# debbiemarkslab/BEAR

Hardware: AMD Instinct MI355X
Metric: k-mer contexts/sec (DM-marginal+grad h), k=13 (higher is better)
Workload: dtype f64

## Files before the change

bear_amd/csrc/bear_hip.hip:

```cpp
#include "bear_host.h"
#include "kernels_finalize.h"
#include "kernels_rows.h"
#include "kernels_sorted.h"
#include "kernels_plan.h"
#include "kernels_synth.h"
#include "kernels_refmix.h"
#include "kernels_mixplan.h"
#include "kernels_sample.h"
#include "kernels_shuffle.h"
#include "kernels_refplan.h"

#ifdef PLN_STAMPS
#define PLN_DBG_ARG , ws->dbg
#else
#define PLN_DBG_ARG
#endif

thread_local int g_last_hip_error = 0;

extern "C" {

int bear_abi_version(void) { return BEAR_ABI_VERSION; }

const char *bear_strerror(int status) {
// ... 648 lines not shown
  hipStream_t s = static_cast<hipStream_t>(stream);
  bear_params only_eps;
  memset(&only_eps, 0, sizeof(only_eps));
  only_eps.eps = eps;
  if (plan_is_rows(plan)) return launch_prior_rows(ws, plan, prior, only_eps, h_signed_dev, train_ar, out, grad_prior, s);
  if (grad_prior) return launch_prior_plan_grad(ws, plan, prior, only_eps, h_signed_dev, train_ar, prior_normalized, out, grad_prior, s);
  return launch_prior_plan(ws, plan, prior, n_rows, only_eps, h_signed_dev, train_ar, prior_normalized, out, s);
}

int bear_dm_refmix_plan_grad_f64(bear_ws *ws, const bear_plan *plan, const uint32_t *counts, const double *net_rows,
                                 const double *ref_rows, uint64_t n_rows, const double *h_signed_dev, const double *tau_signed_dev,
                                 const double *net_weight_signed_dev, double eps, int train_ar, double *out, double *grad_net_rows,
                                 void *stream) {
  int st = check_ws(ws);
  if (st != BEAR_OK) return st;
  if (!plan || !out || !h_signed_dev || !tau_signed_dev || !net_weight_signed_dev) return BEAR_ERR_INVALID_ARG;
  if (n_rows && (!counts || !net_rows || !ref_rows || !grad_net_rows)) return BEAR_ERR_INVALID_ARG;
  if (plan->ncol != 5 || plan->n_rows != n_rows || plan->counts != counts || plan->device != ws->device) return BEAR_ERR_INVALID_ARG;
  if (misaligned(net_rows) || misaligned(ref_rows) || misaligned(grad_net_rows) || misaligned8(out) || misaligned8(h_signed_dev) ||
      misaligned8(tau_signed_dev) || misaligned8(net_weight_signed_dev) || !(eps >= 0.0))
    return BEAR_ERR_INVALID_ARG;
  hipStream_t s = static_cast<hipStream_t>(stream);
  const int grid = grid_plan(ws, plan->n_tiles);
  const double2 *lt = reinterpret_cast<const double2 *>(ws->logtab);
  const pln_view pv = plan_view(plan);
  const bear_step_io io = ws_io(ws, nullptr, BEAR_THETA_REF, out);
  if (train_ar)
    hipLaunchKernelGGL(dm_refmix_plan_grad_kernel<true>, dim3(grid), dim3(PLN_THREADS), sizeof(pln_lds_g), s, net_rows, ref_rows,
                       h_signed_dev, tau_signed_dev, net_weight_signed_dev, eps, pv, lt, grad_net_rows, ws->partials, io);
  else
    hipLaunchKernelGGL(dm_refmix_plan_grad_kernel<false>, dim3(grid), dim3(PLN_THREADS), sizeof(pln_lds_g), s, net_rows, ref_rows,
                       h_signed_dev, tau_signed_dev, net_weight_signed_dev, eps, pv, lt, grad_net_rows, ws->partials, io);
  HIP_TRY(hipGetLastError());
  if (pv.n_heavy_col + pv.n_heavy_row) {
    const uint64_t nh = pv.n_heavy_col + pv.n_heavy_row;
    const int g2 = grid_capped((nh + 255) / 256, (uint64_t)ws->num_cu * 4);
    if (train_ar)
      hipLaunchKernelGGL(dm_refmix_fixup_kernel<true>, dim3(g2), dim3(256), 0, s, net_rows, ref_rows, h_signed_dev, tau_signed_dev,
                         net_weight_signed_dev, eps, pv, lt, grad_net_rows);
    else
      hipLaunchKernelGGL(dm_refmix_fixup_kernel<false>, dim3(g2), dim3(256), 0, s, net_rows, ref_rows, h_signed_dev, tau_signed_dev,
                         net_weight_signed_dev, eps, pv, lt, grad_net_rows);
    HIP_TRY(hipGetLastError());
  }
  return BEAR_OK;
}


static int launch_ref_plan(bear_ws *ws, const bear_plan *plan, const uint32_t *ref, uint64_t n_rows, const bear_params &prm,
                           const double *theta, int train_ar, double *out, hipStream_t s, const bear_apply_io &apply = NO_APPLY) {
  const double2 *lt = reinterpret_cast<const double2 *>(ws->logtab);
  const bear_step_io io = ws_io(ws, theta, BEAR_THETA_REF, out);
  int grid;
  if (plan->rows_ref) {
    if (plan->ref != ref) return BEAR_ERR_INVALID_ARG;
    grid = grid_dense(ws, n_rows);
    if (train_ar)
      hipLaunchKernelGGL(dm_ref_rows_kernel<true>, dim3(grid), dim3(BEAR_THREADS), 0, s, plan->counts, ref, n_rows, prm, lt, ws->partials, io, apply);
    else
      hipLaunchKernelGGL(dm_ref_rows_kernel<false>, dim3(grid), dim3(BEAR_THREADS), 0, s, plan->counts, ref, n_rows, prm, lt, ws->partials, io, apply);
  } else if (plan->ref) {
    if (plan->ref != ref) return BEAR_ERR_INVALID_ARG;
    rpl_view rv;
    rv.items = plan->ref_items;
    rv.n_items = plan->n_ref_items;
    rv.hist0 = plan->hist0;
    rv.heavy0 = plan->heavy0;
    rv.n_heavy0 = plan->n_heavy0;
    rv.sum0 = plan->sum0;
    const uint64_t units = (plan->n_ref_items + 63) / 64, want = (units + 3) / 4 + 2, cap = (uint64_t)ws->num_cu * (units > 131072 ? 6 : 4);
    grid = grid_capped(want, cap);
    if (train_ar)
      hipLaunchKernelGGL(dm_ref_items_kernel<true>, dim3(grid), dim3(256), 0, s, prm, rv, plan_view(plan), lt, ws->partials, io, apply);
    else
      hipLaunchKernelGGL(dm_ref_items_kernel<false>, dim3(grid), dim3(256), 0, s, prm, rv, plan_view(plan), lt, ws->partials, io, apply);
  } else {
    grid = grid_plan(ws, plan->n_tiles);
    if (train_ar)
      hipLaunchKernelGGL(dm_ref_plan_kernel<true>, dim3(grid), dim3(PLN_THREADS), sizeof(pln_lds_r), s, ref, n_rows, prm, plan_view(plan), lt,
                         ws->partials, io, apply);
    else
      hipLaunchKernelGGL(dm_ref_plan_kernel<false>, dim3(grid), dim3(PLN_THREADS), sizeof(pln_lds_r), s, ref, n_rows, prm, plan_view(plan), lt,
                         ws->partials, io, apply);
  }
  HIP_TRY(hipGetLastError());
  (void)grid;
  return BEAR_OK;
}

int bear_dm_ref_plan_f64(bear_ws *ws, const bear_plan *plan, const uint32_t *train, const uint32_t *ref,
                         uint64_t n_rows, double h_signed, double tau_signed, double nu_signed, double eps,
                         int train_ar, double *out, void *stream) {
  int st = check_ws(ws);
  if (st != BEAR_OK) return st;
  if (!plan || !out || (n_rows && (!train || !ref))) return BEAR_ERR_INVALID_ARG;
  if (plan->ncol != 4 || plan->n_rows != n_rows || plan->counts != train || plan->device != ws->device)
    return BEAR_ERR_INVALID_ARG;
  if (misaligned(ref) || (reinterpret_cast<uintptr_t>(out) & 7u)) return BEAR_ERR_INVALID_ARG;
  hipStream_t s = static_cast<hipStream_t>(stream);
  bear_params prm;
  const double tau = exp(tau_signed), nw = exp(nu_signed);
  prm.inv_h = 1.0 / exp(h_signed);
  prm.eps = eps;
  prm.E = exp(-tau);
  prm.tauE = tau * prm.E;
  prm.tau = tau;
  prm.V = 1.0 / (nw + 1.0);
  prm.nw = nw;
  return launch_ref_plan(ws, plan, ref, n_rows, prm, nullptr, train_ar, out, s);
}

int bear_ref_train_reduce_f64(bear_ws *ws, const bear_plan *plan, const uint32_t *train, const uint32_t *ref, uint64_t n_rows,
                              const double *theta, double eps, int train_ar, double *packed, void *stream) {
  int st = check_ws(ws);
  if (st != BEAR_OK) return st;
  if (!plan || !packed || !theta || !n_rows || !train || !ref) return BEAR_ERR_INVALID_ARG;
  if (plan->ncol != 4 || plan->n_rows != n_rows || plan->counts != train || plan->device != ws->device)
    return BEAR_ERR_INVALID_ARG;
  if (misaligned(ref) || (reinterpret_cast<uintptr_t>(packed) & 7u)) return BEAR_ERR_INVALID_ARG;
  hipStream_t s = static_cast<hipStream_t>(stream);
  bear_params only_eps;
  memset(&only_eps, 0, sizeof(only_eps));
  only_eps.eps = eps;
  return launch_ref_plan(ws, plan, ref, n_rows, only_eps, theta, train_ar, packed, s);
}

int bear_ref_train_step_f64(bear_ws *ws, const bear_plan *plan, const uint32_t *train, const uint32_t *ref, uint64_t n_rows,
                            double *theta, double *adam_m, double *adam_v, double *adam_t, double eps, int train_ar,
                            double learning_rate, double scale, double *out, double *loss_buf, uint64_t loss_cap, void *stream) {
  if (!adam_m || !adam_v || !adam_t) return BEAR_ERR_INVALID_ARG;
  if (two_launch_step()) {
    int st = bear_ref_train_reduce_f64(ws, plan, train, ref, n_rows, theta, eps, train_ar, out, stream);
    if (st != BEAR_OK) return st;
    return launch_train_apply(theta, 3, out, adam_m, adam_v, adam_t, learning_rate, scale, train_ar, loss_buf, loss_cap,
                              static_cast<hipStream_t>(stream));
  }
  int st = check_ws(ws);
  if (st != BEAR_OK) return st;
  if (!plan || !out || !theta || !n_rows || !train || !ref) return BEAR_ERR_INVALID_ARG;
  if (plan->ncol != 4 || plan->n_rows != n_rows || plan->counts != train || plan->device != ws->device) return BEAR_ERR_INVALID_ARG;
  if (misaligned(ref) || (reinterpret_cast<uintptr_t>(out) & 7u)) return BEAR_ERR_INVALID_ARG;
  bear_params only_eps;
  memset(&only_eps, 0, sizeof(only_eps));
  only_eps.eps = eps;
  return launch_ref_plan(ws, plan, ref, n_rows, only_eps, theta, train_ar, out, static_cast<hipStream_t>(stream),
                         make_apply(theta, 3, adam_m, adam_v, adam_t, learning_rate, scale, train_ar, loss_buf, loss_cap));
}

int bear_dm_items_f64(bear_ws *ws, const double *x, const uint32_t *c, uint64_t n, int path, double *D, double *P,
                      void *stream) {
  int st = check_ws(ws);
  if (st != BEAR_OK) return st;
  if (n == 0) return BEAR_OK;
  if (!x || !c || !D || !P || path < 0 || path > 2) return BEAR_ERR_INVALID_ARG;
  uint64_t blocks = (n + 255) / 256;
  if (blocks > 0x7fffffffull) return BEAR_ERR_INVALID_ARG;
  hipLaunchKernelGGL(dm_items_kernel, dim3((unsigned)blocks), dim3(256), 0, static_cast<hipStream_t>(stream), x, c, n, path,
                     reinterpret_cast<const double2 *>(ws->logtab), D, P);
  HIP_TRY(hipGetLastError());
  return BEAR_OK;
}

int bear_plan_count_total(const bear_plan *plan, double *total, double *bound) {
  if (!plan) return BEAR_ERR_INVALID_ARG;
  for (int k = 0; k < 3; ++k) {
    if (total) total[k] = plan->count_total[k];
    if (bound) bound[k] = plan->count_bound[k];
  }
  return BEAR_OK;
}

int bear_plan_set_count_bound(bear_plan *plan, const double *bound) {
  if (!plan || !bound) return BEAR_ERR_INVALID_ARG;
  for (int k = 0; k < 3; ++k)
    if (!(bound[k] >= plan->count_total[k]) || !(bound[k] < 0x1p50)) return BEAR_ERR_INVALID_ARG;
  for (int k = 0; k < 3; ++k) plan->count_bound[k] = bound[k];
  return BEAR_OK;
}

static int refmix_grid(const bear_ws *ws, uint64_t n_rows) { return grid_capped((n_rows + RMX_THREADS - 1) / RMX_THREADS, ws_blocks(ws, 2)); }

int bear_ref_mix_forward_f64(bear_ws *ws, const double *net_rows, const double *ref_rows, uint64_t n_rows, const double *tau_signed,
                             const double *net_weight_signed, double *prior, void *stream) {
  int st = check_ws(ws);
  if (st != BEAR_OK) return st;
  if (!tau_signed || !net_weight_signed || misaligned8(tau_signed) || misaligned8(net_weight_signed)) return BEAR_ERR_INVALID_ARG;
  if (n_rows == 0) return BEAR_OK;
  if (!net_rows || !ref_rows || !prior || misaligned(net_rows) || misaligned(ref_rows) || misaligned(prior)) return BEAR_ERR_INVALID_ARG;
  hipLaunchKernelGGL(ref_mix_forward_kernel, dim3(refmix_grid(ws, n_rows)), dim3(RMX_THREADS), 0, static_cast<hipStream_t>(stream),
                     net_rows, ref_rows, tau_signed, net_weight_signed, n_rows, prior);
  HIP_TRY(hipGetLastError());
  return BEAR_OK;
}

int bear_ref_mix_backward_f64(bear_ws *ws, const double *net_rows, const double *ref_rows, const double *grad_prior, uint64_t n_rows,
                              const double *tau_signed, const double *net_weight_signed, double *grad_net_rows, double *grad_scalars,
                              void *stream) {
  int st = check_ws(ws);
  if (st != BEAR_OK) return st;
  if (!tau_signed || !net_weight_signed || !grad_scalars || misaligned8(tau_signed) || misaligned8(net_weight_signed) ||
      misaligned8(grad_scalars))
    return BEAR_ERR_INVALID_ARG;
  hipStream_t s = static_cast<hipStream_t>(stream);
  if (n_rows == 0) {
    HIP_TRY(hipMemsetAsync(grad_scalars, 0, 2 * sizeof(double), s));
    return BEAR_OK;
  }
  if (!net_rows || !ref_rows || !grad_prior || !grad_net_rows || misaligned(net_rows) || misaligned(ref_rows) ||
      misaligned(grad_prior) || misaligned(grad_net_rows))
    return BEAR_ERR_INVALID_ARG;
  hipLaunchKernelGGL(ref_mix_backward_kernel, dim3(refmix_grid(ws, n_rows)), dim3(RMX_THREADS), 0, s, net_rows, ref_rows, grad_prior,
                     tau_signed, net_weight_signed, n_rows, grad_net_rows, ws->partials, ws_arrival(ws), grad_scalars);
  HIP_TRY(hipGetLastError());
  return BEAR_OK;
}

int bear_debug_read_timing(bear_ws *ws, unsigned long long *host, int n_words) {
  if (!ws || !host) return BEAR_ERR_INVALID_ARG;
  HIP_TRY(hipDeviceSynchronize());
  HIP_TRY(hipMemcpy(host, ws->dbg, sizeof(unsigned long long) * (size_t)n_words, hipMemcpyDeviceToHost));
  return BEAR_OK;
}

int bear_debug_occupancy(int which) {
  int nb = -1;
  hipError_t e = which == 0
      ? hipOccupancyMaxActiveBlocksPerMultiprocessor(&nb, dm_prior_sorted_kernel<0>, SRT_THREADS, sizeof(srt_lds_n))
      : hipOccupancyMaxActiveBlocksPerMultiprocessor(&nb, dm_ref_sorted_kernel, SRT_THREADS, sizeof(srt_lds_r));
  return e == hipSuccess ? nb : -1000 - (int)e;
}

int bear_log_gamma_f64(const double *conc, uint64_t n, uint64_t n_samples, uint64_t seed, double *out, void *stream) {
  if (n == 0 || n_samples == 0) return BEAR_OK;
  if (!conc || !out) return BEAR_ERR_INVALID_ARG;
  if (n_samples > (~0ull) / n) return BEAR_ERR_INVALID_ARG;
  const uint64_t total = n * n_samples;
  uint64_t blocks = (total + SMP_THREADS - 1) / SMP_THREADS;
  if (blocks > 65536) blocks = 65536;
  hipLaunchKernelGGL(log_gamma_kernel, dim3((unsigned)blocks), dim3(SMP_THREADS), 0, static_cast<hipStream_t>(stream), conc, n,
                     n_samples, seed, out);
  HIP_TRY(hipGetLastError());
  return BEAR_OK;
}

static int logdir_sample_launch(const uint32_t *counts, const double *prior, uint64_t n_rows, int width, const double *h,
                                int n_h, int with_ar, const double *van, int n_van, int mc_samples, int map, uint64_t seed,
                                uint64_t row_base, double *out, void *stream) {
  if (n_h < 0 || n_van < 0 || n_h + n_van > SMP_MAX_MODELS || (n_h && !h) || (n_van && !van)) return BEAR_ERR_INVALID_ARG;
  if (with_ar && !map) return BEAR_ERR_INVALID_ARG;
  if (map) mc_samples = 1;
  if (mc_samples <= 0) return BEAR_ERR_INVALID_ARG;
  const int M = (with_ar ? 1 : 0) + n_h + n_van;
  if (n_rows == 0 || M == 0) return BEAR_OK;
  if (!out || ((n_h || with_ar) && !prior)) return BEAR_ERR_INVALID_ARG;
  smp_args A;
  memset(&A, 0, sizeof(A));
  A.n_h = n_h;
  A.n_van = n_van;
  A.arm = with_ar ? 1 : 0;
  A.has_counts = counts ? 1 : 0;
  A.has_prior = prior ? 1 : 0;
  A.map = map ? 1 : 0;
  A.mc = (uint32_t)mc_samples;
  A.seed = seed;
  A.row_base = row_base;
  for (int j = 0; j < n_h; ++j) {
    if (!(h[j] > 0.0)) return BEAR_ERR_INVALID_ARG;
    A.w[j] = 1.0 / h[j];
  }
  for (int k = 0; k < n_van; ++k) A.w[n_h + k] = van[k];
  const uint64_t per_row = (uint64_t)M * (uint64_t)mc_samples;
  if (per_row > 0xffffffffull || n_rows > (~0ull) / ((uint64_t)width * per_row)) return BEAR_ERR_INVALID_ARG;
  uint64_t blocks = (n_rows * per_row + SMP_THREADS - 1) / SMP_THREADS;
  if (blocks > 65536) blocks = 65536;
  hipStream_t s = static_cast<hipStream_t>(stream);
  if (width == 21)
    hipLaunchKernelGGL(logdir_sample_kernel<21>, dim3((unsigned)blocks), dim3(SMP_THREADS), 0, s, counts, prior, n_rows, A, out);
  else
    hipLaunchKernelGGL(logdir_sample_kernel<5>, dim3((unsigned)blocks), dim3(SMP_THREADS), 0, s, counts, prior, n_rows, A, out);
  HIP_TRY(hipGetLastError());
  return BEAR_OK;
}

int bear_logdir_sample_f64(const uint32_t *counts, const double *prior, uint64_t n_rows, const double *h, int n_h,
                           int with_ar, const double *van, int n_van, int mc_samples, int map, uint64_t seed,
                           uint64_t row_base, double *out, void *stream) {
  return logdir_sample_launch(counts, prior, n_rows, 5, h, n_h, with_ar, van, n_van, mc_samples, map, seed, row_base, out, stream);
}

int bear_logdir_sample_wide_f64(const uint32_t *counts, const double *prior, uint64_t n_rows, int width, const double *h,
                                int n_h, int with_ar, const double *van, int n_van, int mc_samples, int map, uint64_t seed,
                                uint64_t row_base, double *out, void *stream) {
  if (!wide_width_ok(width)) return BEAR_ERR_INVALID_ARG;
  return logdir_sample_launch(counts, prior, n_rows, width, h, n_h, with_ar, van, n_van, mc_samples, map, seed, row_base, out,
                              stream);
}

int bear_shuffle_rows(const void *src, void *dst, uint64_t n_rows, uint32_t row_bytes, uint64_t seed, void *stream) {
  if (n_rows == 0 || row_bytes == 0) return BEAR_OK;
  if (!src || !dst || src == dst) return BEAR_ERR_INVALID_ARG;
  if (n_rows > (1ull << 62) / row_bytes) return BEAR_ERR_INVALID_ARG;
  const uint32_t hb = shf_half_bits(n_rows);
  const bool words = (row_bytes % 4 == 0) && ((reinterpret_cast<uintptr_t>(src) | reinterpret_cast<uintptr_t>(dst)) % 4 == 0);
  const uint64_t total = words ? n_rows * (row_bytes / 4) : n_rows * (uint64_t)row_bytes;
  uint64_t blocks = (total + 255) / 256;
  if (blocks > 1u << 20) blocks = 1u << 20;
  if (words)
    hipLaunchKernelGGL(shuffle_words_kernel, dim3((unsigned)blocks), dim3(256), 0, static_cast<hipStream_t>(stream),
                       static_cast<const uint32_t *>(src), static_cast<uint32_t *>(dst), n_rows, row_bytes / 4, hb, seed);
// ... 43 lines not shown
```

bear_amd/csrc/bear_math.h:

```cpp
#pragma once
#include <hip/hip_runtime.h>
#include <stdint.h>

#define BEAR_KPROD 16u
#define BEAR_TSTIR 8.0

struct bear_dp {
  double D;
  double P;
};

__device__ __forceinline__ double bear_rcp(double x) {
  double r = __builtin_amdgcn_rcp(x);
  double e = __builtin_fma(-x, r, 1.0);
  r = __builtin_fma(r, e, r);
  e = __builtin_fma(-x, r, 1.0);
  r = __builtin_fma(r, e, r);
  return r;
}

__device__ __forceinline__ double bear_log(double x) { return log(x); }

__device__ __forceinline__ double bear_log1p_pos(double t) {
  double u = 1.0 + t;
  double d = t - (u - 1.0);
  return bear_log(u) + d * bear_rcp(u);
}

__device__ __forceinline__ double bear_stir_lg(double r) {
  double r2 = r * r;
  double s = 1.0 / 156.0;
  s = __builtin_fma(s, r2, -691.0 / 360360.0);
  s = __builtin_fma(s, r2, 1.0 / 1188.0);
  s = __builtin_fma(s, r2, -1.0 / 1680.0);
  s = __builtin_fma(s, r2, 1.0 / 1260.0);
  s = __builtin_fma(s, r2, -1.0 / 360.0);
  s = __builtin_fma(s, r2, 1.0 / 12.0);
  return s * r;
}

__device__ __forceinline__ double bear_stir_psi(double r) {
  double r2 = r * r;
  double s = 1.0 / 12.0;
  s = __builtin_fma(s, r2, -691.0 / 32760.0);
  s = __builtin_fma(s, r2, 1.0 / 132.0);
  s = __builtin_fma(s, r2, -1.0 / 240.0);
  s = __builtin_fma(s, r2, 1.0 / 252.0);
  s = __builtin_fma(s, r2, -1.0 / 120.0);
  s = __builtin_fma(s, r2, 1.0 / 12.0);
  return s * r2;
}

__device__ __forceinline__ bear_dp bear_stirling_diff(double y, double c) {
  double y1 = y + c;
  double ry = bear_rcp(y), ry1 = bear_rcp(y1);
  double l1p = bear_log1p_pos(c * ry);
  double ly = bear_log(y);
  bear_dp o;
  o.D = __builtin_fma(y1 - 0.5, l1p, c * (ly - 1.0)) + (bear_stir_lg(ry1) - bear_stir_lg(ry));
  o.P = l1p - 0.5 * (ry1 - ry) - (bear_stir_psi(ry1) - bear_stir_psi(ry));
  return o;
}

__device__ __forceinline__ bear_dp bear_dm_item(double x, double c) {
  uint32_t m;
  if (c > (double)BEAR_KPROD || x > 0x1p60) {
    double need = BEAR_TSTIR - x;
    m = need > 0.0 ? (uint32_t)ceil(need) : 0u;
  } else {
    m = (uint32_t)c;
  }
  double p = 1.0, dp = 0.0, t = x;
  for (uint32_t j = 0; j < m; ++j) {
    dp = __builtin_fma(dp, t, p);
    p *= t;
    t += 1.0;
  }
  bear_dp o;
  o.D = 0.0;
  o.P = 0.0;
  if (m > 0) {
    o.D = bear_log(p);
    o.P = dp * bear_rcp(p);
  }
  if ((double)m < c) {
    bear_dp s = bear_stirling_diff(t, c - (double)m);
    o.D += s.D;
    o.P += s.P;
  }
  return o;
}

__device__ __forceinline__ double bear_fma3(double a, double b, double c) {
  double r;
  asm("v_fma_f64 %0, %1, %2, %3" : "=v"(r) : "v"(a), "v"(b), "v"(c));
  return r;
}
template <bool COEF_V = false>
__device__ __forceinline__ double bear_log1p_small(double t) {
  double q;
  if (COEF_V) asm("v_fma_f64 %0, %1, %2, %3" : "=v"(q) : "v"(-1.0 / 6.0), "v"(t), "v"(0.2));
  else asm("v_fma_f64 %0, %1, %2, %3" : "=v"(q) : "s"(-1.0 / 6.0), "v"(t), "v"(0.2));
  q = __builtin_fma(q, t, -0.25);
  q = bear_fma3(q, t, 1.0 / 3.0);
  q = __builtin_fma(q, t, -0.5);
  return __builtin_fma(t * t, q, t);
}

#define BEAR_LOGTAB_N 128
template <bool COEF_V = false>
__device__ __forceinline__ double bear_log_tab(double p, const double2 *__restrict__ tab) {
  const double m = __builtin_amdgcn_frexp_mant(p);
  const int e = __builtin_amdgcn_frexp_exp(p);
  const uint32_t hi = (uint32_t)(__double_as_longlong(m) >> 32);
  const double2 rl = tab[(hi >> 13) & 127u];
  const double t = __builtin_fma(m, rl.x, -1.0);
  const double l1p = bear_log1p_small<COEF_V>(t);
  return __builtin_fma((double)e, 0.6931471805599453094, rl.y + l1p);
}


__device__ __forceinline__ bear_dp bear_dm_item_fast(double x, double c, const double2 *__restrict__ tab) {
  uint32_t m;
  const bool stir = c > (double)BEAR_KPROD || x > 0x1p60;
  if (stir) {
    const double need = BEAR_TSTIR - x;
    m = need > 0.0 ? (uint32_t)ceil(need) : 0u;
  } else {
    m = (uint32_t)c;
  }
  double p = 1.0, dp = 0.0, t = x;
  for (uint32_t j = 0; j < m; ++j) {
    dp = __builtin_fma(dp, t, p);
    p *= t;
    t += 1.0;
  }
  bear_dp o;
  o.D = 0.0;
  o.P = 0.0;
  if (m > 0) {
    o.D = bear_log_tab(p, tab);
    o.P = dp * bear_rcp(p);
  }
  if (stir) {
    const double y = t, cc = c - (double)m, y1 = y + cc;
    const double ry = bear_rcp(y), ry1 = bear_rcp(y1);
    const double r = cc * ry;
    const double ly = bear_log_tab(y, tab);
    const double u1 = 1.0 + r;
    const double l1p = r < 0x1p-8 ? bear_log1p_small(r) : __builtin_fma(r - (u1 - 1.0), bear_rcp(u1), bear_log_tab(u1, tab));
    o.D += __builtin_fma(y1 - 0.5, l1p, cc * (ly - 1.0)) + (bear_stir_lg(ry1) - bear_stir_lg(ry));
    o.P += l1p - 0.5 * (ry1 - ry) - (bear_stir_psi(ry1) - bear_stir_psi(ry));
  }
  return o;
}

#define BEAR_EXPTAB_N 128
__device__ __forceinline__ double bear_exp_tab(double z, const double *__restrict__ tab) {
  if (z < -700.0) return 0.0;
  const double kf = __builtin_rint(z * 184.66496523378731);
  double r = __builtin_fma(kf, -0x1.62e42fee00000p-8, z);
  r = __builtin_fma(kf, -0x1.a39ef35793c76p-40, r);
  const int ki = (int)kf;
  const double t = tab[ki & (BEAR_EXPTAB_N - 1)];
  double p = __builtin_fma(r, 1.0 / 120.0, 1.0 / 24.0);
  p = __builtin_fma(r, p, 1.0 / 6.0);
  p = __builtin_fma(r, p, 0.5);
  p = __builtin_fma(r, p, 1.0);
  const double v = __builtin_fma(t, r * p, t);
  return __longlong_as_double(__double_as_longlong(v) + ((long long)(ki >> 7) << 52));
}

template <int CTRL>
__device__ __forceinline__ double bear_dpp_mov(double v) {
  const long long q = __double_as_longlong(v);
  const int lo = __builtin_amdgcn_mov_dpp((int)(uint32_t)q, CTRL, 0xf, 0xf, true);
  const int hi = __builtin_amdgcn_mov_dpp((int)(uint32_t)(q >> 32), CTRL, 0xf, 0xf, true);
  return __longlong_as_double(((long long)hi << 32) | (uint32_t)lo);
}
__device__ __forceinline__ double bear_wave_sum(double v) {
  v += bear_dpp_mov<0xB1>(v);
  v += bear_dpp_mov<0x4E>(v);
  v += bear_dpp_mov<0x124>(v);
  v += bear_dpp_mov<0x128>(v);
#pragma unroll
  for (int step = 0; step < 2; ++step) {
    const long long q = __double_as_longlong(v);
    const uint32_t lo = (uint32_t)q, hi = (uint32_t)(q >> 32);
    const auto a = step == 0 ? __builtin_amdgcn_permlane16_swap(lo, lo, false, false) : __builtin_amdgcn_permlane32_swap(lo, lo, false, false);
    const auto c = step == 0 ? __builtin_amdgcn_permlane16_swap(hi, hi, false, false) : __builtin_amdgcn_permlane32_swap(hi, hi, false, false);
    v = __longlong_as_double(((long long)c[0] << 32) | a[0]) + __longlong_as_double(((long long)c[1] << 32) | a[1]);
  }
  return v;
}
__device__ __forceinline__ double bear_wave_max(double v) {
  v = __builtin_fmax(v, bear_dpp_mov<0xB1>(v));
  v = __builtin_fmax(v, bear_dpp_mov<0x4E>(v));
  v = __builtin_fmax(v, bear_dpp_mov<0x124>(v));
  v = __builtin_fmax(v, bear_dpp_mov<0x128>(v));
#pragma unroll
  for (int step = 0; step < 2; ++step) {
    const long long q = __double_as_longlong(v);
    const uint32_t lo = (uint32_t)q, hi = (uint32_t)(q >> 32);
    const auto a = step == 0 ? __builtin_amdgcn_permlane16_swap(lo, lo, false, false) : __builtin_amdgcn_permlane32_swap(lo, lo, false, false);
    const auto c = step == 0 ? __builtin_amdgcn_permlane16_swap(hi, hi, false, false) : __builtin_amdgcn_permlane32_swap(hi, hi, false, false);
    v = __builtin_fmax(__longlong_as_double(((long long)c[0] << 32) | a[0]), __longlong_as_double(((long long)c[1] << 32) | a[1]));
  }
  return v;
}
```

bear_amd/csrc/kernels_rows.h:

```cpp
#pragma once
#include "bear_common.h"

__device__ __forceinline__ void stage_dwords(uint32_t *lds, const uint32_t *src, uint32_t n_dwords) {
  const uint32_t n_vec = n_dwords >> 2;
  const uint4 *s4 = reinterpret_cast<const uint4 *>(src);
  uint4 *d4 = reinterpret_cast<uint4 *>(lds);
  for (uint32_t i = threadIdx.x; i < n_vec; i += BEAR_THREADS) d4[i] = s4[i];
  for (uint32_t i = (n_vec << 2) + threadIdx.x; i < n_dwords; i += BEAR_THREADS) lds[i] = src[i];
}

__device__ __forceinline__ bear_dp dm_row_item(double x, double c, const double2 *tab) {
  if (tab && x > 0.0 && x < INFINITY) return bear_dm_item_fast(x, c, tab);
  return bear_dm_item(x, c);
}
__device__ __forceinline__ double dm_row(const uint32_t (&c)[5], const double (&a)[5], double (&g)[5], const double2 *tab = nullptr) {
  const double n = (((double)c[0] + (double)c[1]) + ((double)c[2] + (double)c[3])) + (double)c[4];
  double ll = 0.0;
#pragma unroll
  for (int b = 0; b < 5; ++b) g[b] = 0.0;
  if (n == 0.0) return 0.0;
  double A = ((a[0] + a[1]) + (a[2] + a[3])) + a[4];
  bear_dp tn = dm_row_item(A, n, tab);
  ll = -tn.D;
#pragma unroll
  for (int b = 0; b < 5; ++b) {
    g[b] = -tn.P;
    if (c[b] != 0) {
      bear_dp tb = dm_row_item(a[b], (double)c[b], tab);
      ll += tb.D;
      g[b] += tb.P;
    }
  }
  return ll;
}

template <bool AR, bool GRAD>
__global__ __launch_bounds__(BEAR_THREADS) void dm_prior_kernel(const uint32_t *__restrict__ counts,
                                                                 const double *__restrict__ prior,
                                                                 uint64_t n_rows, bear_params prm,
                                                                 double *__restrict__ grad_prior,
                                                                 const double2 *__restrict__ logtab_g,
                                                                 double *__restrict__ partials) {
  __shared__ __attribute__((aligned(16))) uint32_t s_cnt[BEAR_TILE_ROWS * 5];
  __shared__ __attribute__((aligned(16))) double s_pri[BEAR_TILE_ROWS * 5];
  __shared__ double2 s_log[BEAR_LOGTAB_N];
  if (threadIdx.x < BEAR_LOGTAB_N) s_log[threadIdx.x] = logtab_g[threadIdx.x];
  const uint64_t n_tiles = (n_rows + BEAR_TILE_ROWS - 1) / BEAR_TILE_ROWS;
  double acc[2] = {0.0, 0.0};
  for (uint64_t tile = blockIdx.x; tile < n_tiles; tile += gridDim.x) {
    const uint64_t row0 = tile * BEAR_TILE_ROWS;
    const uint32_t rows = (uint32_t)((n_rows - row0 < BEAR_TILE_ROWS) ? (n_rows - row0) : BEAR_TILE_ROWS);
    __syncthreads();
    stage_dwords(s_cnt, counts + row0 * 5, rows * 5);
    stage_dwords(reinterpret_cast<uint32_t *>(s_pri), reinterpret_cast<const uint32_t *>(prior + row0 * 5),
                 rows * 10);
    __syncthreads();
#pragma unroll 1
    for (int k = 0; k < BEAR_ROWS_PER_THREAD; ++k) {
      const uint32_t r = threadIdx.x + k * BEAR_THREADS;
      if (r >= rows) break;
      uint32_t c[5];
      double f[5];
#pragma unroll
      for (int b = 0; b < 5; ++b) {
        c[b] = s_cnt[r * 5 + b];
        f[b] = s_pri[r * 5 + b];
      }
      if (AR) {
#pragma unroll
        for (int b = 0; b < 5; ++b) {
          double p = f[b] + prm.eps;
          double cb = (double)c[b];
          if (c[b] != 0) acc[0] += cb * (p > 0.0 ? bear_log_tab(p, s_log) : bear_log(p));
          if (GRAD) grad_prior[(row0 + r) * 5 + b] = c[b] != 0 ? cb * bear_rcp(p) : 0.0;
        }
      } else {
        double a[5], g[5];
#pragma unroll
        for (int b = 0; b < 5; ++b) a[b] = __builtin_fma(f[b], prm.inv_h, prm.eps);
        acc[0] += dm_row(c, a, g, s_log);
        double dh = 0.0;
#pragma unroll
        for (int b = 0; b < 5; ++b) {
          dh = __builtin_fma(g[b], f[b], dh);
          if (GRAD) grad_prior[(row0 + r) * 5 + b] = g[b] * prm.inv_h;
        }
        acc[1] -= dh * prm.inv_h;
      }
    }
  }
  block_store_partials<2>(acc, partials);
}

#ifndef DPR_TILE_ROWS
#define DPR_TILE_ROWS 512
#endif
#define DPR_BLOCKS_PER_CU 4
template <bool AR, bool GRAD>
__global__ __launch_bounds__(BEAR_THREADS, DPR_BLOCKS_PER_CU / 4) void dm_prior_rows_kernel(const uint32_t *__restrict__ counts, const double *__restrict__ prior,
                                                                      uint64_t n_rows, bear_params prm_arg, double *__restrict__ grad_prior,
                                                                      const double2 *__restrict__ logtab_g, double *__restrict__ partials,
                                                                      const bear_step_io io) {
  __shared__ __attribute__((aligned(16))) uint32_t s_cnt[DPR_TILE_ROWS * 5];
  __shared__ __attribute__((aligned(16))) double s_pri[DPR_TILE_ROWS * 5];
  __shared__ double2 s_log[BEAR_LOGTAB_N];
  const bear_params prm = bear_params_of(prm_arg, io);
  if (threadIdx.x < BEAR_LOGTAB_N) s_log[threadIdx.x] = logtab_g[threadIdx.x];
  const uint64_t n_tiles = (n_rows + DPR_TILE_ROWS - 1) / DPR_TILE_ROWS;
  double acc[2] = {0.0, 0.0};
  for (uint64_t tile = blockIdx.x; tile < n_tiles; tile += gridDim.x) {
    const uint64_t row0 = tile * DPR_TILE_ROWS;
    const uint32_t rows = (uint32_t)((n_rows - row0 < DPR_TILE_ROWS) ? (n_rows - row0) : DPR_TILE_ROWS);
    __syncthreads();
    stage_dwords(s_cnt, counts + row0 * 5, rows * 5);
    stage_dwords(reinterpret_cast<uint32_t *>(s_pri), reinterpret_cast<const uint32_t *>(prior + row0 * 5), rows * 10);
    __syncthreads();
#pragma unroll 1
    for (int k = 0; k < (DPR_TILE_ROWS / BEAR_THREADS); ++k) {
      const uint32_t r = threadIdx.x + k * BEAR_THREADS;
      if (r >= rows) break;
      uint32_t c[5];
      double f[5];
#pragma unroll
      for (int b = 0; b < 5; ++b) {
        c[b] = s_cnt[r * 5 + b];
        f[b] = s_pri[r * 5 + b];
      }
      if (AR) {
#pragma unroll
        for (int b = 0; b < 5; ++b) {
          const double p = f[b] + prm.eps, cb = (double)c[b];
          if (c[b] != 0) acc[0] += cb * (p > 0.0 ? bear_log_tab(p, s_log) : bear_log(p));
          if (GRAD) grad_prior[(row0 + r) * 5 + b] = c[b] != 0 ? cb * bear_rcp(p) : 0.0;
        }
      } else {
        double a[5], g[5];
#pragma unroll
        for (int b = 0; b < 5; ++b) a[b] = __builtin_fma(f[b], prm.inv_h, prm.eps);
        acc[0] += dm_row(c, a, g, s_log);
        double dh = 0.0;
#pragma unroll
        for (int b = 0; b < 5; ++b) {
          dh = __builtin_fma(g[b], f[b], dh);
          if (GRAD) grad_prior[(row0 + r) * 5 + b] = g[b] * prm.inv_h;
        }
        acc[1] -= dh * prm.inv_h;
      }
    }
  }
  __syncthreads();
  block_finish<2>(acc, partials, io);
}

template <bool AR>
__global__ __launch_bounds__(BEAR_THREADS) void dm_ref_kernel(const uint32_t *__restrict__ train,
                                                               const uint32_t *__restrict__ ref,
                                                               uint64_t n_rows, bear_params prm,
                                                               const double2 *__restrict__ logtab_g,
                                                               double *__restrict__ partials) {
  __shared__ double2 s_log[BEAR_LOGTAB_N];
  if (threadIdx.x < BEAR_LOGTAB_N) s_log[threadIdx.x] = logtab_g[threadIdx.x];
  __shared__ __attribute__((aligned(16))) uint32_t s_trn[BEAR_TILE_ROWS * 5];
  __shared__ __attribute__((aligned(16))) uint32_t s_ref[BEAR_TILE_ROWS * 5];
  const uint64_t n_tiles = (n_rows + BEAR_TILE_ROWS - 1) / BEAR_TILE_ROWS;
  double acc[4] = {0.0, 0.0, 0.0, 0.0};
  for (uint64_t tile = blockIdx.x; tile < n_tiles; tile += gridDim.x) {
    const uint64_t row0 = tile * BEAR_TILE_ROWS;
    const uint32_t rows = (uint32_t)((n_rows - row0 < BEAR_TILE_ROWS) ? (n_rows - row0) : BEAR_TILE_ROWS);
    __syncthreads();
    stage_dwords(s_trn, train + row0 * 5, rows * 5);
    stage_dwords(s_ref, ref + row0 * 5, rows * 5);
    __syncthreads();
#pragma unroll 1
    for (int k = 0; k < BEAR_ROWS_PER_THREAD; ++k) {
      const uint32_t r = threadIdx.x + k * BEAR_THREADS;
      if (r >= rows) break;
      uint32_t c[5];
      double rr[4];
#pragma unroll
      for (int b = 0; b < 5; ++b) c[b] = s_trn[r * 5 + b];
#pragma unroll
      for (int b = 0; b < 4; ++b) rr[b] = (double)s_ref[r * 5 + b] + prm.eps;
      const double invR = bear_rcp((rr[0] + rr[1]) + (rr[2] + rr[3]));
      double f[5], dft[5], dfn[5];
#pragma unroll
      for (int b = 0; b < 4; ++b) {
        double dev = __builtin_fma(rr[b], invR, -0.25);
        f[b] = __builtin_fma(prm.E, dev, 0.25) * prm.V;
        dft[b] = -prm.tauE * dev * prm.V;
        dfn[b] = -prm.nw * f[b] * prm.V;
      }
      f[4] = prm.nw * prm.V;
      dft[4] = 0.0;
      dfn[4] = prm.nw * (1.0 - f[4]) * prm.V;
      double dLdf[5];
      if (AR) {
#pragma unroll
        for (int b = 0; b < 5; ++b) {
          double p = f[b] + prm.eps;
          double cb = (double)c[b];
          dLdf[b] = 0.0;
          if (c[b] != 0) {
            acc[0] += cb * (p > 0.0 ? bear_log_tab(p, s_log) : bear_log(p));
            dLdf[b] = cb * bear_rcp(p);
          }
        }
      } else {
        double a[5], g[5];
#pragma unroll
        for (int b = 0; b < 5; ++b) a[b] = __builtin_fma(f[b], prm.inv_h, prm.eps);
        acc[0] += dm_row(c, a, g);
        double dh = 0.0;
#pragma unroll
        for (int b = 0; b < 5; ++b) {
          dLdf[b] = g[b] * prm.inv_h;
          dh = __builtin_fma(dLdf[b], f[b], dh);
        }
        acc[1] -= dh;
      }
#pragma unroll
      for (int b = 0; b < 5; ++b) {
        acc[2] = __builtin_fma(dLdf[b], dft[b], acc[2]);
        acc[3] = __builtin_fma(dLdf[b], dfn[b], acc[3]);
      }
    }
  }
  block_store_partials<4>(acc, partials);
}

template <bool AR>
__global__ __launch_bounds__(BEAR_THREADS) void dm_ref_rows_kernel(const uint32_t *__restrict__ train, const uint32_t *__restrict__ ref,
                                                                    uint64_t n_rows, bear_params prm_arg, const double2 *__restrict__ logtab_g,
                                                                    double *__restrict__ partials, const bear_step_io io,
                                                                    const bear_apply_io apply) {
  __shared__ double2 s_log[BEAR_LOGTAB_N];
  __shared__ __attribute__((aligned(16))) uint32_t s_trn[DPR_TILE_ROWS * 5];
  __shared__ __attribute__((aligned(16))) uint32_t s_ref[DPR_TILE_ROWS * 5];
  const bear_params prm = bear_params_of(prm_arg, io);
  if (threadIdx.x < BEAR_LOGTAB_N) s_log[threadIdx.x] = logtab_g[threadIdx.x];
  const uint64_t n_tiles = (n_rows + DPR_TILE_ROWS - 1) / DPR_TILE_ROWS;
  double acc[4] = {0.0, 0.0, 0.0, 0.0};
  for (uint64_t tile = blockIdx.x; tile < n_tiles; tile += gridDim.x) {
    const uint64_t row0 = tile * DPR_TILE_ROWS;
    const uint32_t rows = (uint32_t)((n_rows - row0 < DPR_TILE_ROWS) ? (n_rows - row0) : DPR_TILE_ROWS);
    __syncthreads();
    stage_dwords(s_trn, train + row0 * 5, rows * 5);
    stage_dwords(s_ref, ref + row0 * 5, rows * 5);
    __syncthreads();
#pragma unroll 1
    for (int k = 0; k < DPR_TILE_ROWS / BEAR_THREADS; ++k) {
      const uint32_t r = threadIdx.x + k * BEAR_THREADS;
      if (r >= rows) break;
      uint32_t c[5];
      double rr[4];
#pragma unroll
      for (int b = 0; b < 5; ++b) c[b] = s_trn[r * 5 + b];
#pragma unroll
      for (int b = 0; b < 4; ++b) rr[b] = (double)s_ref[r * 5 + b] + prm.eps;
      const double invR = bear_rcp((rr[0] + rr[1]) + (rr[2] + rr[3]));
      double f[5], dft[5], dfn[5];
#pragma unroll
      for (int b = 0; b < 4; ++b) {
        const double dev = __builtin_fma(rr[b], invR, -0.25);
        f[b] = __builtin_fma(prm.E, dev, 0.25) * prm.V;
        dft[b] = -prm.tauE * dev * prm.V;
        dfn[b] = -prm.nw * f[b] * prm.V;
      }
      f[4] = prm.nw * prm.V;
      dft[4] = 0.0;
      dfn[4] = prm.nw * (1.0 - f[4]) * prm.V;
      double dLdf[5];
      if (AR) {
#pragma unroll
        for (int b = 0; b < 5; ++b) {
          const double p = f[b] + prm.eps, cb = (double)c[b];
          dLdf[b] = 0.0;
          if (c[b] != 0) {
            acc[0] += cb * (p > 0.0 ? bear_log_tab(p, s_log) : bear_log(p));
            dLdf[b] = cb * bear_rcp(p);
          }
        }
      } else {
        double a[5], g[5];
#pragma unroll
        for (int b = 0; b < 5; ++b) a[b] = __builtin_fma(f[b], prm.inv_h, prm.eps);
        acc[0] += dm_row(c, a, g, s_log);
        double dh = 0.0;
#pragma unroll
        for (int b = 0; b < 5; ++b) {
          dLdf[b] = g[b] * prm.inv_h;
          dh = __builtin_fma(dLdf[b], f[b], dh);
        }
        acc[1] -= dh;
      }
#pragma unroll
      for (int b = 0; b < 5; ++b) {
        acc[2] = __builtin_fma(dLdf[b], dft[b], acc[2]);
        acc[3] = __builtin_fma(dLdf[b], dfn[b], acc[3]);
      }
    }
  }
  __syncthreads();
  block_finish<4>(acc, partials, io, apply);
}
```

Measured before the change: 141.0 billion.

## Add wave-uniform dense Dirichlet-multinomial path with shared row term and adaptive Stirling terms

Adds a dense fast path for DM row likelihoods. It is taken when every count in the wave exceeds the product threshold and every alpha is in range. The path uses a merged product-log per row, reuses a precomputed lgamma/digamma of the shared total alpha when the prior sums to one, and shortens the Stirling series based on the wave's minimum argument. Sparse rows go through a noinline call, and the prior and ref kernels are restructured to compute cells lazily in a rolled loop with sched barriers. Launch bounds are raised to target more waves per SIMD. The extra ballot logic and the branchy, less-unrolled structure could cost something on mixed waves.

After: 140.4 billion. Within noise of the previous version (-0.5%).

```diff
diff --git a/bear_amd/csrc/bear_hip.hip b/bear_amd/csrc/bear_hip.hip
--- a/bear_amd/csrc/bear_hip.hip
+++ b/bear_amd/csrc/bear_hip.hip
@@ -824,9 +824,15 @@
   int st = check_ws(ws);
   if (st != BEAR_OK) return st;
   if (n == 0) return BEAR_OK;
-  if (!x || !c || !D || !P || path < 0 || path > 2) return BEAR_ERR_INVALID_ARG;
+  if (!x || !c || !D || !P || path < 0 || path > 3) return BEAR_ERR_INVALID_ARG;
   uint64_t blocks = (n + 255) / 256;
   if (blocks > 0x7fffffffull) return BEAR_ERR_INVALID_ARG;
+  if (path == 3) {
+    hipLaunchKernelGGL(dm_dense_items_kernel<0>, dim3((unsigned)blocks), dim3(256), 0, static_cast<hipStream_t>(stream), x, c, n,
+                       reinterpret_cast<const double2 *>(ws->logtab), D, P);
+    HIP_TRY(hipGetLastError());
+    return BEAR_OK;
+  }
   hipLaunchKernelGGL(dm_items_kernel, dim3((unsigned)blocks), dim3(256), 0, static_cast<hipStream_t>(stream), x, c, n, path,
                      reinterpret_cast<const double2 *>(ws->logtab), D, P);
   HIP_TRY(hipGetLastError());
diff --git a/bear_amd/csrc/bear_math.h b/bear_amd/csrc/bear_math.h
--- a/bear_amd/csrc/bear_math.h
+++ b/bear_amd/csrc/bear_math.h
@@ -152,6 +152,115 @@
     o.D += __builtin_fma(y1 - 0.5, l1p, cc * (ly - 1.0)) + (bear_stir_lg(ry1) - bear_stir_lg(ry));
     o.P += l1p - 0.5 * (ry1 - ry) - (bear_stir_psi(ry1) - bear_stir_psi(ry));
   }
+  return o;
+}
+
+#define BEAR_DENSE_XMIN 0x1p-100
+#define BEAR_DENSE_XMAX 0x1p30
+#define BEAR_HALF_LOG_2PI 0.91893853320467274178
+
+__device__ __forceinline__ double bear_stir_lg_nt(double r, int nt) {
+  const double r2 = r * r;
+  double s = -1.0 / 360.0;
+  if (nt > 2) {
+    double q = -1.0 / 1680.0;
+    if (nt > 4) {
+      q = 1.0 / 156.0;
+      q = __builtin_fma(q, r2, -691.0 / 360360.0);
+      q = __builtin_fma(q, r2, 1.0 / 1188.0);
+      q = __builtin_fma(q, r2, -1.0 / 1680.0);
+    }
+    q = __builtin_fma(q, r2, 1.0 / 1260.0);
+    s = __builtin_fma(q, r2, -1.0 / 360.0);
+  }
+  s = __builtin_fma(s, r2, 1.0 / 12.0);
+  return s * r;
+}
+__device__ __forceinline__ double bear_stir_psi_nt(double r, int nt) {
+  const double r2 = r * r;
+  double s = -1.0 / 120.0;
+  if (nt > 2) {
+    double q = -1.0 / 240.0;
+    if (nt > 4) {
+      q = 1.0 / 12.0;
+      q = __builtin_fma(q, r2, -691.0 / 32760.0);
+      q = __builtin_fma(q, r2, 1.0 / 132.0);
+      q = __builtin_fma(q, r2, -1.0 / 240.0);
+    }
+    q = __builtin_fma(q, r2, 1.0 / 252.0);
+    s = __builtin_fma(q, r2, -1.0 / 120.0);
+  }
+  s = __builtin_fma(s, r2, 1.0 / 12.0);
+  return s * r2;
+}
+__device__ __forceinline__ void bear_dense_cell(double x, double c, int nt, const double2 *__restrict__ tab, double &p_out, double &D, double &P) {
+  const double need = BEAR_TSTIR - x;
+  const double cc = c - (need > 0.0 ? __builtin_ceil(need) : 0.0);
+  double p = 1.0, dp = 0.0, t = x;
+#pragma unroll 1
+  while (t < BEAR_TSTIR) {
+    dp = __builtin_fma(dp, t, p);
+    p *= t;
+    t += 1.0;
+  }
+  const double y = t, y1 = y + cc;
+  const double py = p * y;
+  const double rq = bear_rcp(py * y1);
+  const double ry1 = rq * py, ty = rq * y1;
+  const double ry = ty * p, rp = ty * y;
+  const double ly = bear_log_tab(y, tab);
+  double l1p, M;
+  if (cc >= y) {
+    const double ly1 = bear_log_tab(y1, tab);
+    l1p = ly1 - ly;
+    M = __builtin_fma(y1 - 0.5, ly1, -__builtin_fma(y - 0.5, ly, cc));
+  } else {
+    const double r = cc * ry, u1 = 1.0 + r;
+    l1p = r < 0x1p-8 ? bear_log1p_small(r) : __builtin_fma(r - (u1 - 1.0), bear_rcp(u1), bear_log_tab(u1, tab));
+    M = __builtin_fma(y1 - 0.5, l1p, cc * (ly - 1.0));
+  }
+  p_out = p;
+  D = M + (bear_stir_lg_nt(ry1, nt) - bear_stir_lg(ry));
+  P = __builtin_fma(dp, rp, l1p - 0.5 * (ry1 - ry) - (bear_stir_psi_nt(ry1, nt) - bear_stir_psi(ry)));
+}
+
+__device__ __forceinline__ bear_dp bear_lgamma_psi(double A) {
+  const double need = BEAR_TSTIR - A;
+  const uint32_t m = need > 0.0 ? (uint32_t)ceil(need) : 0u;
+  double p = 1.0, dp = 0.0, t = A;
+  for (uint32_t j = 0; j < m; ++j) {
+    dp = __builtin_fma(dp, t, p);
+    p *= t;
+    t += 1.0;
+  }
+  const double ry = bear_rcp(t), ly = bear_log(t);
+  bear_dp o;
+  o.D = (__builtin_fma(t - 0.5, ly, -t) + BEAR_HALF_LOG_2PI) + bear_stir_lg(ry);
+  o.P = ly - 0.5 * ry - bear_stir_psi(ry);
+  if (m > 0) {
+    o.D -= bear_log(p);
+    o.P -= dp * bear_rcp(p);
+  }
+  return o;
+}
+struct bear_dense_const {
+  double A, lgA, psiA;
+  bool ok;
+};
+__device__ __forceinline__ bear_dense_const bear_dense_const_of(double u, double eps) {
+  bear_dense_const k;
+  k.A = u + 5.0 * eps;
+  k.ok = k.A >= BEAR_DENSE_XMIN && k.A < BEAR_DENSE_XMAX;
+  const bear_dp o = bear_lgamma_psi(k.ok ? k.A : 1.0);
+  k.lgA = o.D;
+  k.psiA = o.P;
+  return k;
+}
+__device__ __forceinline__ bear_dp bear_dense_rowterm(const bear_dense_const &k, double n, int nt, const double2 *__restrict__ tab) {
+  const double y1 = k.A + n, ry1 = bear_rcp(y1), l = bear_log_tab(y1, tab);
+  bear_dp o;
+  o.D = ((__builtin_fma(y1 - 0.5, l, -y1) + BEAR_HALF_LOG_2PI) + bear_stir_lg_nt(ry1, nt)) - k.lgA;
+  o.P = (l - 0.5 * ry1 - bear_stir_psi_nt(ry1, nt)) - k.psiA;
   return o;
 }
 
diff --git a/bear_amd/csrc/kernels_rows.h b/bear_amd/csrc/kernels_rows.h
--- a/bear_amd/csrc/kernels_rows.h
+++ b/bear_amd/csrc/kernels_rows.h
@@ -13,25 +13,88 @@
   if (tab && x > 0.0 && x < INFINITY) return bear_dm_item_fast(x, c, tab);
   return bear_dm_item(x, c);
 }
+__device__ __noinline__ bear_dp dm_row_item_call(double x, double c, const double2 *tab) { return dm_row_item(x, c, tab); }
+template <bool CALL = false>
+__device__ __forceinline__ double dm_row_cells(const uint32_t (&c)[5], const double (&a)[5], const bear_dp &tn, double (&g)[5], const double2 *tab) {
+  double ll = -tn.D;
+#pragma unroll
+  for (int b = 0; b < 5; ++b) {
+    g[b] = -tn.P;
+    if (c[b] != 0) {
+      bear_dp tb = CALL ? dm_row_item_call(a[b], (double)c[b], tab) : dm_row_item(a[b], (double)c[b], tab);
+      ll += tb.D;
+      g[b] += tb.P;
+    }
+  }
+  return ll;
+}
 __device__ __forceinline__ double dm_row(const uint32_t (&c)[5], const double (&a)[5], double (&g)[5], const double2 *tab = nullptr) {
   const double n = (((double)c[0] + (double)c[1]) + ((double)c[2] + (double)c[3])) + (double)c[4];
-  double ll = 0.0;
 #pragma unroll
   for (int b = 0; b < 5; ++b) g[b] = 0.0;
   if (n == 0.0) return 0.0;
   double A = ((a[0] + a[1]) + (a[2] + a[3])) + a[4];
-  bear_dp tn = dm_row_item(A, n, tab);
-  ll = -tn.D;
-#pragma unroll
+  return dm_row_cells(c, a, dm_row_item(A, n, tab), g, tab);
+}
+
+#define DM_DENSE_XMIN_HI 0x39B00000u
+#define DM_DENSE_XMAX_HI 0x41D00000u
+__device__ __forceinline__ uint32_t dm_hi32(double v) { return (uint32_t)((unsigned long long)__double_as_longlong(v) >> 32); }
+__device__ __forceinline__ bool dm_dense_ok(const uint32_t (&c)[5], const double (&a)[5]) {
+  bool ok = true;
+#pragma unroll
+  for (int b = 0; b < 5; ++b) ok = ok && c[b] > BEAR_KPROD && dm_hi32(a[b]) >= DM_DENSE_XMIN_HI && dm_hi32(a[b]) < DM_DENSE_XMAX_HI;
+  return ok;
+}
+__device__ __forceinline__ bool dm_wave_dense(const uint32_t (&c)[5], const double (&a)[5]) {
+  return __builtin_amdgcn_ballot_w64(!dm_dense_ok(c, a)) == 0ull;
+}
+__device__ __forceinline__ int dm_wave_terms(const uint32_t (&c)[5], const double (&a)[5]) {
+  double ymin = a[0] + (double)c[0];
+#pragma unroll
+  for (int b = 1; b < 5; ++b) ymin = __builtin_fmin(ymin, a[b] + (double)c[b]);
+  const uint32_t hi = dm_hi32(ymin);
+  if (__builtin_amdgcn_ballot_w64(hi < 0x40900000u) == 0ull) return 2;
+  if (__builtin_amdgcn_ballot_w64(hi < 0x40500000u) == 0ull) return 4;
+  return 7;
+}
+template <bool DENSE, class Cell, class Sink>
+__device__ __forceinline__ double dm_ctx(double n, double A_own, bool shared, const bear_dense_const &K, int nt, const double2 *tab,
+                                         Cell &&cell, Sink &&sink) {
+  bear_dp tn = {0.0, 0.0};
+  if (DENSE && shared && n >= K.A) tn = bear_dense_rowterm(K, n, nt, tab);
+  else if (DENSE || n != 0.0) tn = dm_row_item_call(A_own, n, tab);
+  double ll = DENSE ? 0.0 : -tn.D, pp = 1.0;
+#pragma unroll 1
   for (int b = 0; b < 5; ++b) {
-    g[b] = -tn.P;
-    if (c[b] != 0) {
-      bear_dp tb = dm_row_item(a[b], (double)c[b], tab);
-      ll += tb.D;
-      g[b] += tb.P;
-    }
-  }
-  return ll;
+    uint32_t cb;
+    double ab;
+    cell(b, cb, ab);
+    if (DENSE) {
+      double p, D, P;
+      bear_dense_cell(ab, (double)cb, nt, tab, p, D, P);
+      pp *= p;
+      ll += D;
+      sink(b, P - tn.P);
+    } else {
+      double gb = n != 0.0 ? -tn.P : 0.0;
+      if (cb != 0) {
+        const bear_dp tb = dm_row_item_call(ab, (double)cb, tab);
+        ll += tb.D;
+        gb += tb.P;
+      }
+      sink(b, gb);
+    }
+    __builtin_amdgcn_sched_barrier(0);
+  }
+  return DENSE ? (ll + bear_log_tab(pp, tab)) - tn.D : ll;
+}
+__device__ __forceinline__ bear_dense_const dm_dense_const(const bear_params &prm) {
+  bear_dense_const K = bear_dense_const_of(prm.inv_h, prm.eps);
+  K.A = bear_uniform_f64(K.A);
+  K.lgA = bear_uniform_f64(K.lgA);
+  K.psiA = bear_uniform_f64(K.psiA);
+  return K;
 }
 
 template <bool AR, bool GRAD>
@@ -96,8 +159,10 @@
 #define DPR_TILE_ROWS 512
 #endif
 #define DPR_BLOCKS_PER_CU 4
+#define DPR_WAVES_PER_SIMD (DPR_BLOCKS_PER_CU * (BEAR_THREADS / 64) / 4)
+#define DPR_SUM1_TOL 4.5e-16
 template <bool AR, bool GRAD>
-__global__ __launch_bounds__(BEAR_THREADS, DPR_BLOCKS_PER_CU / 4) void dm_prior_rows_kernel(const uint32_t *__restrict__ counts, const double *__restrict__ prior,
+__global__ __launch_bounds__(BEAR_THREADS, DPR_WAVES_PER_SIMD) void dm_prior_rows_kernel(const uint32_t *__restrict__ counts, const double *__restrict__ prior,
                                                                       uint64_t n_rows, bear_params prm_arg, double *__restrict__ grad_prior,
                                                                       const double2 *__restrict__ logtab_g, double *__restrict__ partials,
                                                                       const bear_step_io io) {
@@ -105,6 +170,8 @@
   __shared__ __attribute__((aligned(16))) double s_pri[DPR_TILE_ROWS * 5];
   __shared__ double2 s_log[BEAR_LOGTAB_N];
   const bear_params prm = bear_params_of(prm_arg, io);
+  bear_dense_const K = {};
+  if (!AR) K = dm_dense_const(prm);
   if (threadIdx.x < BEAR_LOGTAB_N) s_log[threadIdx.x] = logtab_g[threadIdx.x];
   const uint64_t n_tiles = (n_rows + DPR_TILE_ROWS - 1) / DPR_TILE_ROWS;
   double acc[2] = {0.0, 0.0};
@@ -134,16 +201,27 @@
           if (GRAD) grad_prior[(row0 + r) * 5 + b] = c[b] != 0 ? cb * bear_rcp(p) : 0.0;
         }
       } else {
-        double a[5], g[5];
+        double a[5];
 #pragma unroll
         for (int b = 0; b < 5; ++b) a[b] = __builtin_fma(f[b], prm.inv_h, prm.eps);
-        acc[0] += dm_row(c, a, g, s_log);
-        double dh = 0.0;
-#pragma unroll
-        for (int b = 0; b < 5; ++b) {
-          dh = __builtin_fma(g[b], f[b], dh);
-          if (GRAD) grad_prior[(row0 + r) * 5 + b] = g[b] * prm.inv_h;
-        }
+        const bool dense = dm_wave_dense(c, a);
+        const double n = (((double)c[0] + (double)c[1]) + ((double)c[2] + (double)c[3])) + (double)c[4];
+        const double A_own = ((a[0] + a[1]) + (a[2] + a[3])) + a[4];
+        const bool shared = K.ok && __builtin_fabs((((f[0] + f[1]) + (f[2] + f[3])) + f[4]) - 1.0) <= DPR_SUM1_TOL;
+        const int nt = dense ? dm_wave_terms(c, a) : 7;
+        asm volatile("" ::: "memory");
+        double dh = 0.0, fb;
+        auto cell = [&](int b, uint32_t &cb, double &ab) {
+          cb = s_cnt[r * 5 + b];
+          fb = s_pri[r * 5 + b];
+          ab = __builtin_fma(fb, prm.inv_h, prm.eps);
+        };
+        auto sink = [&](int b, double gb) {
+          dh = __builtin_fma(gb, fb, dh);
+          if (GRAD) grad_prior[(row0 + r) * 5 + b] = gb * prm.inv_h;
+        };
+        if (dense) acc[0] += dm_ctx<true>(n, A_own, shared, K, nt, s_log, cell, sink);
+        else acc[0] += dm_ctx<false>(n, A_own, shared, K, nt, s_log, cell, sink);
         acc[1] -= dh * prm.inv_h;
       }
     }
@@ -229,7 +307,7 @@
 }
 
 template <bool AR>
-__global__ __launch_bounds__(BEAR_THREADS) void dm_ref_rows_kernel(const uint32_t *__restrict__ train, const uint32_t *__restrict__ ref,
+__global__ __launch_bounds__(BEAR_THREADS, DPR_WAVES_PER_SIMD) void dm_ref_rows_kernel(const uint32_t *__restrict__ train, const uint32_t *__restrict__ ref,
                                                                     uint64_t n_rows, bear_params prm_arg, const double2 *__restrict__ logtab_g,
                                                                     double *__restrict__ partials, const bear_step_io io,
                                                                     const bear_apply_io apply) {
@@ -237,6 +315,8 @@
   __shared__ __attribute__((aligned(16))) uint32_t s_trn[DPR_TILE_ROWS * 5];
   __shared__ __attribute__((aligned(16))) uint32_t s_ref[DPR_TILE_ROWS * 5];
   const bear_params prm = bear_params_of(prm_arg, io);
+  bear_dense_const K = {};
+  if (!AR) K = dm_dense_const(prm);
   if (threadIdx.x < BEAR_LOGTAB_N) s_log[threadIdx.x] = logtab_g[threadIdx.x];
   const uint64_t n_tiles = (n_rows + DPR_TILE_ROWS - 1) / DPR_TILE_ROWS;
   double acc[4] = {0.0, 0.0, 0.0, 0.0};
@@ -269,8 +349,8 @@
       f[4] = prm.nw * prm.V;
       dft[4] = 0.0;
       dfn[4] = prm.nw * (1.0 - f[4]) * prm.V;
-      double dLdf[5];
       if (AR) {
+        double dLdf[5];
 #pragma unroll
         for (int b = 0; b < 5; ++b) {
           const double p = f[b] + prm.eps, cb = (double)c[b];
@@ -280,26 +360,72 @@
             dLdf[b] = cb * bear_rcp(p);
           }
         }
+#pragma unroll
+        for (int b = 0; b < 5; ++b) {
+          acc[2] = __builtin_fma(dLdf[b], dft[b], acc[2]);
+          acc[3] = __builtin_fma(dLdf[b], dfn[b], acc[3]);
+        }
       } else {
-        double a[5], g[5];
+        double a[5];
 #pragma unroll
         for (int b = 0; b < 5; ++b) a[b] = __builtin_fma(f[b], prm.inv_h, prm.eps);
-        acc[0] += dm_row(c, a, g, s_log);
-        double dh = 0.0;
-#pragma unroll
-        for (int b = 0; b < 5; ++b) {
-          dLdf[b] = g[b] * prm.inv_h;
-          dh = __builtin_fma(dLdf[b], f[b], dh);
-        }
+        const bool dense = dm_wave_dense(c, a);
+        const double n = (((double)c[0] + (double)c[1]) + ((double)c[2] + (double)c[3])) + (double)c[4];
+        const double A_own = ((a[0] + a[1]) + (a[2] + a[3])) + a[4];
+        const int nt = dense ? dm_wave_terms(c, a) : 7;
+        asm volatile("" ::: "memory");
+        double dh = 0.0, fb, dev;
+        auto cell = [&](int b, uint32_t &cb, double &ab) {
+          cb = s_trn[r * 5 + b];
+          if (b < 4) {
+            dev = __builtin_fma((double)s_ref[r * 5 + b] + prm.eps, invR, -0.25);
+            fb = __builtin_fma(prm.E, dev, 0.25) * prm.V;
+          } else {
+            dev = 0.0;
+            fb = prm.nw * prm.V;
+          }
+          ab = __builtin_fma(fb, prm.inv_h, prm.eps);
+        };
+        auto sink = [&](int b, double gb) {
+          const double dl = gb * prm.inv_h;
+          dh = __builtin_fma(dl, fb, dh);
+          const double dt = b < 4 ? -prm.tauE * dev * prm.V : 0.0;
+          const double dn = b < 4 ? -prm.nw * fb * prm.V : prm.nw * (1.0 - fb) * prm.V;
+          acc[2] = __builtin_fma(dl, dt, acc[2]);
+          acc[3] = __builtin_fma(dl, dn, acc[3]);
+        };
+        if (dense) acc[0] += dm_ctx<true>(n, A_own, K.ok, K, nt, s_log, cell, sink);
+        else acc[0] += dm_ctx<false>(n, A_own, K.ok, K, nt, s_log, cell, sink);
         acc[1] -= dh;
-      }
-#pragma unroll
-      for (int b = 0; b < 5; ++b) {
-        acc[2] = __builtin_fma(dLdf[b], dft[b], acc[2]);
-        acc[3] = __builtin_fma(dLdf[b], dfn[b], acc[3]);
       }
     }
   }
   __syncthreads();
   block_finish<4>(acc, partials, io, apply);
 }
+
+template <int UNIT = 0>
+__global__ __launch_bounds__(256) void dm_dense_items_kernel(const double *__restrict__ x, const uint32_t *__restrict__ c, uint64_t n,
+                                                             const double2 *__restrict__ logtab_g, double *__restrict__ D,
+                                                             double *__restrict__ P) {
+  __shared__ double2 s_log[BEAR_LOGTAB_N];
+  if (threadIdx.x < BEAR_LOGTAB_N) s_log[threadIdx.x] = logtab_g[threadIdx.x];
+  __syncthreads();
+  const uint64_t i = (uint64_t)blockIdx.x * 256 + threadIdx.x;
+  if (i >= n) return;
+  const double xi = x[i];
+  const uint32_t ci = c[i];
+  const bool in = ci > BEAR_KPROD && dm_hi32(xi) >= DM_DENSE_XMIN_HI && dm_hi32(xi) < DM_DENSE_XMAX_HI;
+  const double y1 = in ? xi + (double)ci : INFINITY;
+  const int nt = __builtin_amdgcn_ballot_w64(!(y1 >= 0x1p10)) == 0ull ? 2 : (__builtin_amdgcn_ballot_w64(!(y1 >= 0x1p6)) == 0ull ? 4 : 7);
+  bear_dp o = {0.0, 0.0};
+  if (in) {
+    double p;
+    bear_dense_cell(xi, (double)ci, nt, s_log, p, o.D, o.P);
+    o.D += bear_log_tab(p, s_log);
+  } else if (ci != 0) {
+    o = xi > 0.0 ? dm_row_item_call(xi, (double)ci, s_log) : bear_dp{__builtin_nan(""), __builtin_nan("")};
+  }
+  D[i] = o.D;
+  P[i] = o.P;
+}
```
